# chao1224/pytorch_distributed_nn

Measured on AMD Instinct MI355X. Metric: samples/sec (whole node) ResNet-50 DDP, higher is better.
Workload: dtype bf16; 1 GPU; model=resnet50 (ImageNet layout, 224x224, 1000 classes), global_batch=256, per_gpu_batch=256, image_size=224, parallelism=dp1, optimizer=fused SGD momentum=0.9 wd=5e-5, hipgraph=False, opt_overlap=False

## Files before the change

csrc/kernels/conv1x1_wide.hip:

```cpp
#include "conv_direct.h"

namespace {
using namespace pg;

enum { PRE_NONE = 0, PRE_GM = 1 };
constexpr int W1_NB = 64;

template <int EPI, int PRE>
__global__ void __launch_bounds__(256, 2) conv1x1_wide_kernel(C3Args a) {
    constexpr int NB = W1_NB, FN = NB / 16;
    constexpr int BPT = NB * 8 / 256;
    extern __shared__ __attribute__((aligned(16))) char smem[];
    bf16_t* const bbuf = reinterpret_cast<bf16_t*>(smem);
    float* const coef = reinterpret_cast<float*>(bbuf + 2 * NB * 64);
    const int tid = threadIdx.x, lane = tid & 63, wave = tid >> 6;
    const int groups = a.ntiles;
    const int t = xcd_remap(blockIdx.x, a.tiles * groups);
    const int tile = t / groups, nt = t - tile * groups;
    const int p0 = tile * C3_BM, n0 = nt * NB;
    const int K = a.C, KC = K >> 6;

    u16x8_t rb[BPT];
    auto load_b = [&](int kc) {
#pragma unroll
// ... 105 lines not shown
}

template <int EPI, int PRE>
int wide_launch(const C3Args& a, hipStream_t st) {
    const int sm = 2 * W1_NB * 128 + (PRE != PRE_NONE ? 3 * a.C * 4 : 0);
    hipLaunchKernelGGL((conv1x1_wide_kernel<EPI, PRE>), dim3(a.tiles * a.ntiles), dim3(256), sm, st, a);
    PDNN_LAUNCH_RET;
}

template <int PRE>
int wide_dispatch(const C3Args& a, int epi, hipStream_t st) {
    switch (epi) {
        case C3_BNB: return wide_launch<C3_BNB, PRE>(a, st);
        case C3_STATS: return wide_launch<C3_STATS, PRE>(a, st);
        case C3_RES: return wide_launch<C3_RES, PRE>(a, st);
        default: return wide_launch<C3_PLAIN, PRE>(a, st);
    }
}

}

static FastDiv w1_fdiv(uint32_t d) {
    FastDiv f;
    f.d = d ? d : 1;
    uint32_t l = 0;
    while ((1ull << l) < f.d) ++l;
    f.s = l;
    f.m = (uint32_t)((((1ull << l) - f.d) << 32) / f.d + 1);
    return f;
}
// ... 14 lines not shown
    a.x = x; a.w = w; a.y = y; a.C = K; a.N = N; a.P = (int)P;
    a.dW = w1_fdiv(1); a.dH = w1_fdiv(1);
    a.stats = stats; a.res = res; a.rmask = res_mask;
    a.ep_x = bn_x; a.ep_mean = bn_mean; a.ep_invstd = bn_invstd; a.ep_mscale = bn_mscale; a.ep_mshift = bn_mshift;
    a.pre_t = pre_t; a.pre_mean = pre_mean; a.pre_invstd = pre_invstd; a.pre_gamma = pre_gamma;
    a.pre_dgamma = pre_dgamma; a.pre_dbeta = pre_dbeta; a.pre_out = pre_out;
    if (pre_t && !(pre_mean && pre_invstd && pre_dgamma && pre_dbeta)) return (int)hipErrorInvalidValue;
    if (pre_out && !pre_t) return (int)hipErrorInvalidValue;
    if (bn_x && !(bn_mean && bn_invstd && bn_mscale && bn_mshift)) return (int)hipErrorInvalidValue;
    const int epi = bn_x ? C3_BNB : (stats ? C3_STATS : (res ? C3_RES : C3_PLAIN));
    a.tiles = (int)cdiv(P, C3_BM);
    a.ntiles = N / W1_NB;
    if (pre_t) return wide_dispatch<PRE_GM>(a, epi, st);
    return wide_dispatch<PRE_NONE>(a, epi, st);
}
```

csrc/kernels/conv3x3.hip:

```cpp
#include "conv_direct.h"

namespace {
using namespace pg;

typedef __attribute__((ext_vector_type(8))) int c3v8i;
typedef __attribute__((ext_vector_type(4))) int c3v4i;
constexpr int C3_AMAX_PARTS = 1024;
#ifndef C3_PRE_J
#define C3_PRE_J 3
#endif
#ifndef C3_F8_PRE_J
#define C3_F8_PRE_J 2
#endif

template <int FMT>
__device__ __forceinline__ uint4 c3_to_fp8(const float* v) {
    constexpr float MX = FMT ? 57344.f : 448.f;
    int w[4];
#pragma unroll
    for (int d = 0; d < 4; ++d) {
        const float c0 = fminf(fmaxf(v[4 * d], -MX), MX), c1 = fminf(fmaxf(v[4 * d + 1], -MX), MX);
        const float c2 = fminf(fmaxf(v[4 * d + 2], -MX), MX), c3 = fminf(fmaxf(v[4 * d + 3], -MX), MX);
        int x = 0;
        if constexpr (FMT) {
// ... 616 lines not shown
}

template <int KC, int NB, bool PRE>
int areg_dispatch(const C3Args& a, int epi, hipStream_t st) {
    if constexpr (!PRE) {
        if (a.pro_sc) {
            if (epi == C3_STATS) return areg_launch<KC, NB, C3_STATS, false, true>(a, st);
            if (epi == C3_PLAIN) return areg_launch<KC, NB, C3_PLAIN, false, true>(a, st);
            return (int)hipErrorInvalidValue;
        }
    }
    switch (epi) {
        case C3_BNB: return areg_launch<KC, NB, C3_BNB, PRE>(a, st);
        case C3_STATS: return areg_launch<KC, NB, C3_STATS, PRE>(a, st);
        case C3_RES: return areg_launch<KC, NB, C3_RES, PRE>(a, st);
        default: return areg_launch<KC, NB, C3_PLAIN, PRE>(a, st);
    }
}

template <bool PRE>
int areg_run(C3Args& a, int K, int epi, hipStream_t st) {
    const int nb = K == 256 ? 32 : 64;
    const int chunks = a.N / nb;
    int g = 1;
    while (g < chunks && (long)a.tiles * g < 512 && chunks % (2 * g) == 0) g *= 2;
    a.ntiles = g;
    if (K == 64) return areg_dispatch<1, 64, PRE>(a, epi, st);
    if (K == 128) return areg_dispatch<2, 64, PRE>(a, epi, st);
    return areg_dispatch<4, 32, PRE>(a, epi, st);
}

static bool set_pre(C3Args& a, const bf16_t* t, const float* mean, const float* invstd, const float* gamma,
             const float* dgamma, const float* dbeta, bf16_t* out) {
    a.pre_t = t; a.pre_mean = mean; a.pre_invstd = invstd; a.pre_gamma = gamma;
    a.pre_dgamma = dgamma; a.pre_dbeta = dbeta; a.pre_out = out;
    if (!t) return !out;
    return mean && invstd && dgamma && dbeta;
}
static int c3_force() { return pg::tune().conv3x3_force; }

static FastDiv make_fdiv_c3(uint32_t d) {
    FastDiv f;
// ... 143 lines not shown
    if (!pdnn_conv1x1_panel_supported(P, K, N) || (bn_x && !stats) || (res_mask && !res) || (!pro_sc != !pro_sh) ||
        (pro_sc && (pre_t || bn_x || res)))
        return (int)hipErrorInvalidValue;
    C3Args a{};
    a.x = x; a.w = w; a.y = y; a.C = K; a.N = N; a.P = (int)P;
    a.tiles = (int)cdiv(P, C3_BM);
    a.stats = stats; a.res = res; a.rmask = res_mask;
    a.ep_x = bn_x; a.ep_mean = bn_mean; a.ep_invstd = bn_invstd; a.ep_mscale = bn_mscale; a.ep_mshift = bn_mshift;
    if (!set_pre(a, pre_t, pre_mean, pre_invstd, pre_gamma, pre_dgamma, pre_dbeta, pre_out))
        return (int)hipErrorInvalidValue;
    a.pro_sc = pro_sc; a.pro_sh = pro_sh;
    const int epi = bn_x ? C3_BNB : (stats ? C3_STATS : (res ? C3_RES : C3_PLAIN));
    return pre_t ? areg_run<true>(a, K, epi, st) : areg_run<false>(a, K, epi, st);
}

PDNN_API int pdnn_conv1x1_panel_stats_rows(long P) { return (int)cdiv(P, C3_BM) * 4; }
```

csrc/kernels/conv_direct.h:

```cpp
#pragma once
#include "gemm_common.h"
#include "tuning.h"

namespace {
using namespace pg;

constexpr int C3_BM = 256;
enum { C3_PLAIN = 0, C3_STATS = 1, C3_BNB = 2, C3_RES = 3 };

struct C3Args {
    const bf16_t* x;
    const bf16_t* w;
    bf16_t* y;
    int Nimg, H, W, C, N, P;
    FastDiv dW, dH;
    int tiles, ntiles;
    int halo_max;
    float* stats;
    const bf16_t* res;
    const uint8_t* rmask;
    const bf16_t* ep_x;
    const float *ep_mean, *ep_invstd, *ep_mscale, *ep_mshift;
    const bf16_t* pre_t;
    const float *pre_mean, *pre_invstd, *pre_gamma, *pre_dgamma, *pre_dbeta;
    bf16_t* pre_out;
    const float *f8_scale, *f8_inv, *f8_winv;
    float* f8_amax;
    const float *pro_sc, *pro_sh;
};

struct PreCoef {
    float k[8], A[8], B[8];
};
__device__ __forceinline__ void pre_coef(const C3Args& a, int c, PreCoef& pc) {
    const float invL = (float)(1.0 / (double)a.P);
// ... 68 lines not shown
    u.x &= m; u.y &= m; u.z &= m; u.w &= m;
    return __builtin_bit_cast(u16x8_t, u);
}

__device__ __forceinline__ u16x8_t c3_zero8() {
    u16x8_t z = {0, 0, 0, 0, 0, 0, 0, 0};
    return z;
}

__device__ __forceinline__ int halo_off(int hp, int q) {
    return hp * 64 + ((q ^ ((hp >> 1) & 7)) << 3);
}

template <int NB, int EPI>
struct C3PairOps {
    static constexpr bool RES = EPI == C3_RES, BNB = EPI == C3_BNB;
    u16x4_t tv[(RES || BNB) ? 2 : 1][4];
    uint32_t mw[RES ? 4 : 1];
};

template <int NB, int EPI>
__device__ __forceinline__ void c3_load_pair(const C3Args& a, const long (&lrow)[4], int n0, int lg, int fp,
                                             C3PairOps<NB, EPI>& o) {
    constexpr bool RES = EPI == C3_RES, BNB = EPI == C3_BNB;
    if constexpr (RES) {
#pragma unroll
        for (int fm = 0; fm < 4; ++fm)
            o.mw[fm] = a.rmask ? *reinterpret_cast<const uint32_t*>(a.rmask + ((lrow[fm] + n0 + 32 * fp) >> 3))
                               : 0xFFFFFFFFu;
    }
    if constexpr (RES || BNB) {
        const bf16_t* src = BNB ? a.ep_x : a.res;
#pragma unroll
        for (int h = 0; h < 2; ++h) {
            const int n = n0 + (2 * fp + h) * 16 + 4 * lg;
#pragma unroll
            for (int fm = 0; fm < 4; ++fm) o.tv[h][fm] = *reinterpret_cast<const u16x4_t*>(src + lrow[fm] + n);
        }
    }
}

template <int NB, int EPI>
__device__ __forceinline__ void c3_epilogue_rows(const C3Args& a, f32x4_t (&acc)[4][NB / 16], int tile,
                                                 const long (&orow)[4], int n0, int wave, int lane,
                                                 const bool (&pv)[4]) {
    constexpr int FN = NB / 16, NP = FN / 2;
    constexpr bool RES = EPI == C3_RES;
    const int lg = lane >> 4;
    long lrow[4];
#pragma unroll
    for (int fm = 0; fm < 4; ++fm) lrow[fm] = pv[fm] ? orow[fm] : 0;
    C3PairOps<NB, EPI> cur, nxt;
    if constexpr (NP > 1) c3_load_pair<NB, EPI>(a, lrow, n0, lg, 0, cur);
    else if constexpr (RES) {
#pragma unroll
        for (int fm = 0; fm < 4; ++fm)
            cur.mw[fm] = a.rmask ? *reinterpret_cast<const uint32_t*>(a.rmask + ((lrow[fm] + n0) >> 3)) : 0xFFFFFFFFu;
    }
#pragma unroll
    for (int fp = 0; fp < NP; ++fp) {
        if (fp + 1 < NP) c3_load_pair<NB, EPI>(a, lrow, n0, lg, fp + 1, nxt);
        uint32_t pk[4][2][2];
#pragma unroll
        for (int h = 0; h < 2; ++h) {
            const int fn = 2 * fp + h;
            const int n = n0 + fn * 16 + 4 * lg;
            float s[4] = {0, 0, 0, 0}, q[4] = {0, 0, 0, 0};
            float bms[4], bmh[4];
            if constexpr (NP == 1 && (RES || EPI == C3_BNB)) {
                const bf16_t* src = EPI == C3_BNB ? a.ep_x : a.res;
#pragma unroll
                for (int fm = 0; fm < 4; ++fm)
                    cur.tv[h][fm] = pv[fm] ? *reinterpret_cast<const u16x4_t*>(src + orow[fm] + n) : u16x4_t{0, 0, 0, 0};
            }
            if constexpr (EPI == C3_BNB) {
                const float4 m4 = *reinterpret_cast<const float4*>(a.ep_mscale + n);
                const float4 h4 = *reinterpret_cast<const float4*>(a.ep_mshift + n);
                bms[0] = m4.x; bms[1] = m4.y; bms[2] = m4.z; bms[3] = m4.w;
                bmh[0] = h4.x; bmh[1] = h4.y; bmh[2] = h4.z; bmh[3] = h4.w;
            }
#pragma unroll
            for (int fm = 0; fm < 4; ++fm) {
                const bool ok = pv[fm];
                float v[4];
#pragma unroll
                for (int j = 0; j < 4; ++j) v[j] = acc[fm][fn][j];
                if constexpr (RES) {
                    const uint32_t mb = cur.mw[fm] >> (16 * h + 4 * lg);
#pragma unroll
                    for (int j = 0; j < 4; ++j) v[j] += ((mb >> j) & 1) ? bf2f(cur.tv[h][fm][j]) : 0.f;
                }
                if constexpr (EPI == C3_BNB) {
#pragma unroll
                    for (int j = 0; j < 4; ++j) {
                        const float tt = bf2f(cur.tv[h][fm][j]);
                        const float gm = (ok && fmaf(tt, bms[j], bmh[j]) > 0.f) ? bf2f(f2bf(v[j])) : 0.f;
                        v[j] = gm;
                        s[j] += gm;
                        q[j] += gm * tt;
                    }
                } else if constexpr (EPI == C3_STATS) {
                    if (ok) {
#pragma unroll
                        for (int j = 0; j < 4; ++j) {
                            const float r = bf2f(f2bf(v[j]));
                            s[j] += r;
                            q[j] += r * r;
                        }
                    }
                }
                pk[fm][h][0] = pk2bf(v[0], v[1]);
                pk[fm][h][1] = pk2bf(v[2], v[3]);
            }
            if constexpr (EPI == C3_STATS || EPI == C3_BNB) {
#pragma unroll
                for (int j = 0; j < 4; ++j) {
                    s[j] = row16_sum(s[j]);
                    q[j] = row16_sum(q[j]);
                }
                {
                    float* ps = stat_row(a.stats, (long)tile * 4 + wave, a.N) + n;
                    if constexpr (EPI == C3_BNB) {
                        const int j = lane & 3;
                        if ((lane & 12) == 4) {
                            const float qj = (sel4(q, j) - a.ep_mean[n + j] * sel4(s, j)) * a.ep_invstd[n + j];
                            q[0] = q[1] = q[2] = q[3] = qj;
                        }
                    }
                    stat_add_frag(ps, ps + a.N, lane, s, q, true);
                }
            }
        }
#pragma unroll
        for (int fm = 0; fm < 4; ++fm) {
            const auto s0 = __builtin_amdgcn_permlane16_swap(pk[fm][0][0], pk[fm][1][0], false, false);
            const auto s1 = __builtin_amdgcn_permlane16_swap(pk[fm][0][1], pk[fm][1][1], false, false);
            const int n = n0 + (2 * fp + (lg & 1)) * 16 + 8 * (lg >> 1);
            if (pv[fm]) *reinterpret_cast<uint4*>(a.y + orow[fm] + n) = make_uint4(s0[0], s1[0], s0[1], s1[1]);
        }
        if (fp + 1 < NP) cur = nxt;
// ... 14 lines not shown
```

pytorch_distributed_nn_amd/ops/_backend.py:

```python
from __future__ import annotations

import ctypes
import functools
import os
from pathlib import Path

import torch

_LIBDIR = Path(__file__).resolve().parent.parent / "_lib"
_LIB = None
_ERR = None

P = ctypes.c_void_p
I = ctypes.c_int
L = ctypes.c_long
F = ctypes.c_float
D = ctypes.c_double

_SIGS = {
    "pdnn_gemm_nt": [P, L, P, L, P, L, I, I, I, F, P, I, I, P],
    "pdnn_gemm_nn": [P, L, P, L, P, L, I, I, I, F, I, P],
    "pdnn_gemm_tn_acc": [P, L, P, L, P, L, I, I, I, F, P],
    "pdnn_conv_fwd": [P, P, P, I, I, I, I, I, I, I, I, I, I, I, P, P, P, P],
    "pdnn_conv_dgrad": [P, P, P, I, I, I, I, I, I, I, I, I, I, I, P, P, P, P, P, P, P, P, P],
# ... 17 lines not shown
    "pdnn_conv3x3_wgrad_supported": [I, I, I, I, I],
    "pdnn_conv3x3_wgrad_ws": [I, I, I, I, I],
    "pdnn_conv3x3_force": [I],
    "pdnn_tune_set": [ctypes.c_char_p, I],
    "pdnn_tune_get": [ctypes.c_char_p],
    "pdnn_tune_list": [ctypes.c_char_p, I],
    "pdnn_tune_error": [],
    "pdnn_tune_unknown": [],
    "pdnn_set_comm_world": [I],
    "pdnn_grid_cus": [],
    "pdnn_conv1x1_panel": [P, P, P, L, I, I, P, P, P, P, P, P, P, P, P, P, P, P, P, P, P, P, P, P],
    "pdnn_conv1x1_panel_supported": [L, I, I],
    "pdnn_conv1x1_panel_stats_rows": [L],
    "pdnn_conv1x1_wide": [P, P, P, L, I, I] + [P] * 16,
    "pdnn_conv1x1_wide_supported": [L, I, I],
    "pdnn_stem_conv": [P, P, P, I, I, I, I, I, P, P],
    "pdnn_stem_stats_rows": [L],
    "pdnn_stem_conv_nchw": [P, P, P, I, I, I, I, I, P, P],
    "pdnn_stem_wgrad_nchw": [P, P, P, I, I, I, I, I, P, P, P, P, P, P, P, P, P, P, P],
    "pdnn_stem_wgrad_ws": [I, I, I],
    "pdnn_bn_relu_maxpool": [P, P, P, P, P, I, I, I, I, I, I, P],
    "pdnn_set_glds_mode": [I],
    "pdnn_set_pp_mode": [I],
    "pdnn_set_pp_bn": [I],
    "pdnn_set_pp_trace": [P],
    "pdnn_pp_wgrad": [P, L, P, L, P, L, I, I, I, F, P, I, P, I, P],
    "pdnn_pp_wgrad_plan": [I, I, I, I],
    "pdnn_pp_wgrad_splits": [I, I, I],
    "pdnn_pp_wgrad_ws": [I, I, I],
    "pdnn_pp_wgrad_splits_long": [I, I, I],
# ... 188 lines not shown
```

pytorch_distributed_nn_amd/ops/fused_resnet.py:

```python
from __future__ import annotations

import contextlib
import os

import torch

from .. import tuning
from ..optim.flat import SHADOW_EPOCH, direct_grad, grad_ready
from . import kernels as K
from .functional import weight_bf16

F32 = torch.float32


def _bn_train(slab, M, bn_params, bufs, mom, eps):
    gamma, beta = bn_params
    rm, rv = bufs
    rows = slab.shape[0] // 2
    return K.bn_finalize(slab, rows, M, eps, mom, gamma, beta, rm, rv)


def _bn_eval(bn_params, bufs, eps):
    gamma, beta = bn_params
    rm, rv = bufs
# ... 140 lines not shown


def _bn_back(g2d, t2d, mean, inv, gamma, mode, msrc=None, msc=None, msh=None, sink=None, bn_params=None):
    slab, _, rows = K.bn_bwd_reduce(g2d, t2d, mean, inv, mode=mode, msrc=msrc, mscale=msc, mshift=msh)
    if sink is not None:
        (dgamma, dbeta), (rg, rb) = sink.bn(slab, rows, *bn_params)
        dt, _, _ = K.bn_bwd_apply(g2d, t2d, mean, inv, gamma, dgamma, dbeta, mode=mode, msrc=msrc, mscale=msc,
                                  mshift=msh)
        return dt, rg, rb
    dgamma, dbeta = K.bn_bwd_finalize(slab, rows)
    dt, _, _ = K.bn_bwd_apply(g2d, t2d, mean, inv, gamma, dgamma, dbeta, mode=mode, msrc=msrc, mscale=msc,
                              mshift=msh)
    return dt, dgamma, dbeta


def _dgrad_bn_gm(dy, wk, t, st, pad, mean, inv, sc, sh, sink, gamma_p, beta_p, wprep=None):
    gm, slab = K.conv_dgrad(dy, wk, t.shape, st, pad, bn=(t, mean, inv, sc, sh), wprep=wprep)
    (dgamma, dbeta), ret = sink.bn(slab, slab.shape[0] // 2, gamma_p, beta_p)
    return gm, dgamma, dbeta, ret


_FWD_FORKED = {}
_WPREP_SEQ = [0]
_WPREP_WAITED = {}


@contextlib.contextmanager
def side_forward(dev):
    side = _side_stream(dev) if dev.type == "cuda" else None
    if side is None:
        yield
        return
    K.stream_wait(side, torch.cuda.current_stream(dev))
    _FWD_FORKED[dev.index] = SHADOW_EPOCH[0]
    try:
        yield
    finally:
        _FWD_FORKED.pop(dev.index, None)


def _wait_wprep(dev, ev, seq):
    if _WPREP_WAITED.get(dev.index, -1) >= seq:
        return
# ... 17 lines not shown
        ev.record(side)
    for sp, w in zip(specs, ws):
        if sp is None:
            continue
        sp[1].record_stream(side)
        if w is not None:
            w.record_stream(main)
    _WPREP_SEQ[0] += 1
    return ws, (ev, _WPREP_SEQ[0])


def _pre_ok(t, wk, st, pad):
    return K.dgrad_pre_ok(tuple(t.shape), tuple(wk.shape), st, pad)


def _fused_dgrad_bn(dy, wk, t, st, pad, mean, inv, sc, sh, gamma, sink, gamma_p, beta_p, wprep=None):
    gm, slab = K.conv_dgrad(dy, wk, t.shape, st, pad, bn=(t, mean, inv, sc, sh), wprep=wprep)
    (dgamma, dbeta), ret = sink.bn(slab, slab.shape[0] // 2, gamma_p, beta_p)
    C = t.shape[-1]
    dt, _, _ = K.bn_bwd_apply(gm.view(-1, C), t.view(-1, C), mean, inv, gamma, dgamma, dbeta, mode=0)
    return dt.view(t.shape), ret[0], ret[1]


def _krsc_grad(dw):
    return dw.permute(0, 3, 1, 2)


class BottleneckFn(torch.autograd.Function):

    @staticmethod
    def forward(ctx, x, conf, bufs, shadows, *params):
        stride, training, mom, eps = conf[:4]
        fp8_meta = conf[4] if len(conf) > 4 else None
        down = len(params) == 12
        w1, g1, b1, w2, g2, b2, w3, g3, b3 = params[:9]
        k1, k2, k3 = shadows[:3]
        side_down = None
        xd = x
        side = _side_stream(x.device) if down else None
        if side is not None:
            main = torch.cuda.current_stream(x.device)
            K.stream_wait(side, main)
            with torch.cuda.stream(side):
                side_down, xd = _shortcut_fwd(x, shadows[3], stride, training, (params[10], params[11]), bufs[6:8],
                                              mom, eps)
            x.record_stream(side)
            for t in side_down + (xd,):
                t.record_stream(main)
        t1, m1, i1, s1, h1 = _conv_bn(x, k1, 1, 0, None, training, (g1, b1), bufs[0:2], mom, eps)
        C1 = t1.shape[-1]
        if stride == 1 and K.conv3x3_pro_ok(tuple(t1.shape), w2.shape[0]):
# ... 29 lines not shown
        t3, m3, i3, s3, h3 = _conv_bn(src2, k3, 1, 0, pro2, training, (g3, b3), bufs[4:6], mom, eps)
        C3 = t3.shape[-1]
        if down:
            if side_down is not None:
                K.stream_wait(main, side)
                td, md, idd, sd, hd = side_down
            else:
                (td, md, idd, sd, hd), xd = _shortcut_fwd(x, shadows[3], stride, training, (params[10], params[11]),
                                                          bufs[6:8], mom, eps)
            out, mb = K.bn_apply(t3.view(-1, C3), s3, h3, res=td.view(-1, C3), rscale=sd, rshift=hd, relu=True,
                                 want_mask=training)
        else:
            td = md = idd = None
            out, mb = K.bn_apply(t3.view(-1, C3), s3, h3, res=x.view(-1, C3), relu=True, want_mask=training)
        out = out.view(t3.shape)
        ctx.wprep = None
        if training:
            ctx.wprep = _prep_dgrad_weights(x, [(tuple(t3.shape), k3, tuple(t2.shape), 1, 0),
                                                (tuple(t2.shape), k2, tuple(t1.shape), stride, 1) if fp8 is None
                                                else None,
                                                (tuple(t1.shape), k1, tuple(x.shape), 1, 0)])
        ctx.save_for_backward(x, t1, a1, t2, t3, td, mb, m1, i1, s1, h1, m2, i2, s2, h2, m3, i3, md, idd,
                              g1, g2, g3, params[10] if down else None, k1, k2, k3, shadows[3] if down else None, a2,
                              xd if (down and xd is not x) else None)
        ctx.conf = (stride, training, down)
        ctx.params = params
        ctx.fp8 = fp8
        return out

    @staticmethod
    def backward(ctx, gout):
        (x, t1, a1, t2, t3, td, mb, m1, i1, s1, h1, m2, i2, s2, h2, m3, i3, md, idd,
         g1, g2, g3, gd, k1, k2, k3, kd, a2, xs) = ctx.saved_tensors
        stride, training, down = ctx.conf
        if not training:
            raise RuntimeError("fused Bottleneck backward requires training-mode BatchNorm")
        gout = gout.contiguous()
        C3 = t3.shape[-1]
        g2d, t3_2d = gout.view(-1, C3), t3.view(-1, C3)
        P = ctx.params
        ctx.params = None
        sink = _Sink(gout.device)
        w3p = w2p = w1p = None
        if ctx.wprep is not None:
            (w3p, w2p, w1p), (ev, seq) = ctx.wprep
            _wait_wprep(gout.device, ev, seq)
            ctx.wprep = None
        gres_mask = mb if MASKED_RES else None
        slab3, slabd, rows = K.bn_bwd_reduce(g2d, t3_2d, m3, i3, mode=3, msrc=mb,
                                             x2=td.view(-1, C3) if down else None, mean2=md, invstd2=idd)
        (dg3, db3), (rg3, rb3) = sink.bn(slab3, rows, P[7], P[8])
        if down:
            (dgd, dbd), (rgd, rbd) = sink.bn(slabd, rows, P[10], P[11])
            dt3, dtd, _ = K.bn_bwd_apply(g2d, t3_2d, m3, i3, g3, dg3, db3, mode=3, msrc=mb,
                                         x2=td.view(-1, C3), mean2=md, invstd2=idd, gamma2=gd, dgamma2=dgd,
                                         dbeta2=dbd)
            gres = None
        elif MASKED_RES:
            dt3, _, _ = K.bn_bwd_apply(g2d, t3_2d, m3, i3, g3, dg3, db3, mode=3, msrc=mb)
            gres = gout
        else:
            dt3, _, gres = K.bn_bwd_apply(g2d, t3_2d, m3, i3, g3, dg3, db3, mode=3, msrc=mb, want_gm=True)
        dt3 = dt3.view(t3.shape)
        dw3 = sink.wgrad(P[6], a2 if a2 is not None else t2, dt3, 1, 1, 1, 0, pro=None if a2 is not None else (s2, h2))
        bn1 = (t1, m1, i1, s1, h1)
        if _pre_ok(t2, k2, stride, 1):
            gm2, dg2, db2, (rg2, rb2) = _dgrad_bn_gm(dt3, k3, t2, 1, 0, m2, i2, s2, h2, sink, P[4], P[5], wprep=w3p)
            dt2 = torch.empty_like(t2)
            pre2 = (t2, m2, i2, g2, dg2, db2, dt2)
            if ctx.fp8 is not None:
                from .fp8 import weight_fp8_flip
                wt8, winv = weight_fp8_flip(P[3])
                gm1, slab1 = K.conv3x3_fp8(gm2, wt8, winv, ctx.fp8.bwd, bn=bn1, pre=pre2)
            else:
                gm1, slab1 = K.conv_dgrad(gm2, k2, t1.shape, stride, 1, bn=bn1, pre=pre2, wprep=w2p)
            del gm2
            dw2 = sink.wgrad(P[3], a1 if a1 is not None else t1, dt2, 3, 3, stride, 1,
                             pro=None if a1 is not None else (s1, h1), fp8=ctx.fp8)
        else:
            dt2, rg2, rb2 = _fused_dgrad_bn(dt3, k3, t2, 1, 0, m2, i2, s2, h2, g2, sink, P[4], P[5], wprep=w3p)
            dw2 = sink.wgrad(P[3], a1 if a1 is not None else t1, dt2, 3, 3, stride, 1,
                             pro=None if a1 is not None else (s1, h1))
            gm1, slab1 = K.conv_dgrad(dt2, k2, t1.shape, stride, 1, bn=bn1, wprep=w2p)
        (dg1, db1), (rg1, rb1) = sink.bn(slab1, slab1.shape[0] // 2, P[1], P[2])
        pre1 = None
        if _pre_ok(t1, k1, 1, 0):
            dt1 = torch.empty_like(t1)
            pre1 = (t1, m1, i1, g1, dg1, db1, dt1)
            dy1 = gm1
        else:
            C1 = t1.shape[-1]
            dt1 = K.bn_bwd_apply(gm1.view(-1, C1), t1.view(-1, C1), m1, i1, g1, dg1, db1, mode=0)[0].view(t1.shape)
            dw1 = sink.wgrad(P[0], x, dt1, 1, 1, 1, 0)
            dy1 = dt1
        if down:
            dtd = dtd.view(td.shape)
            dwd = sink.wgrad(P[9], xs, dtd, 1, 1, 1, 0) if xs is not None else sink.wgrad(P[9], x, dtd, 1, 1, stride, 0)
            dx = K.conv_dgrad(dy1, k1, x.shape, 1, 0, pre=pre1, wprep=w1p)
            dx = K.conv_dgrad(dtd, kd, x.shape, stride, 0, res=dx, out=dx)
        else:
            dx = K.conv_dgrad(dy1, k1, x.shape, 1, 0, res=gres.view(x.shape), res_mask=gres_mask, pre=pre1,
                              wprep=w1p)
        if pre1 is not None:
            dw1 = sink.wgrad(P[0], x, dt1, 1, 1, 1, 0)
        grads = (dw1, rg1, rb1, dw2, rg2, rb2, dw3, rg3, rb3) + ((dwd, rgd, rbd) if down else ())
        sink.done()
        return (dx, None, None, None) + grads


class BasicBlockFn(torch.autograd.Function):

    @staticmethod
    def forward(ctx, x, conf, bufs, shadows, *params):
        stride, training, mom, eps = conf
# ... 162 lines not shown
```

pytorch_distributed_nn_amd/ops/kernels.py:

```python
from __future__ import annotations

import ctypes

import torch

from ._backend import _CUR_DEV, call, lib, ptr, stream

BF16 = torch.bfloat16
F32 = torch.float32


def _chk(cond, msg):
    if not cond:
        raise ValueError(msg)


def _is_krsc(w):
    K, C, R, S = w.shape
    return w.stride() == (R * S * C, 1, S * C, C)


def _bf16_c(t, name):
    _chk(t.dtype == BF16 and t.is_cuda, f"{name}: expected CUDA bf16, got {t.dtype} {t.device}")
    _chk(t.is_contiguous(), f"{name}: expected contiguous tensor")
# ... 238 lines not shown
    return (_P1["mode"] and R == 1 and S == 1 and st == 1 and pad == 0
            and (lib().pdnn_conv1x1_panel_supported(P, K, N) == 1 or _wide_ok(P, K, N, fwd)))


def _pre_args(pre, x):
    if pre is None:
        return (None,) * 7
    t, mean, inv, gamma, dg, db, dt_out = pre
    _bf16_c(t, "pre.t")
    _chk(t.numel() == x.numel(), "pre: t must have the operand's shape")
    if dt_out is not None:
        _chk(dt_out.numel() == x.numel() and dt_out.dtype == BF16 and dt_out.is_contiguous(), "pre: dt_out")
    return tuple(ptr(v) for v in (t, mean, inv, gamma, dg, db, dt_out))


def conv1x1_panel(x2d, w2d, want_stats=False, res=None, bn=None, res_mask=None, out=None, pre=None, pro=None):
    P, Kc = x2d.shape
    N = w2d.shape[0]
    y = out if out is not None else torch.empty(P, N, device=x2d.device, dtype=BF16)
    slab = None
    t = mean = inv = msc = msh = None
    if want_stats or bn is not None:
        slab = stat_bins(N, x2d.device)
    if bn is not None:
        t, mean, inv, msc, msh = bn
    if Kc >= 512:
        _chk(pro is None, "conv1x1_panel: the forward prologue needs K <= 256")
        call("pdnn_conv1x1_wide", ptr(x2d), ptr(w2d), ptr(y), P, Kc, N, ptr(slab), ptr(res), ptr(res_mask), ptr(t),
             ptr(mean), ptr(inv), ptr(msc), ptr(msh), *_pre_args(pre, x2d), stream())
        return y, slab
    psc, psh = pro if pro is not None else (None, None)
    call("pdnn_conv1x1_panel", ptr(x2d), ptr(w2d), ptr(y), P, Kc, N, ptr(slab), ptr(res), ptr(res_mask), ptr(t),
         ptr(mean), ptr(inv), ptr(msc), ptr(msh), *_pre_args(pre, x2d), ptr(psc), ptr(psh), stream())
    return y, slab
# ... 57 lines not shown


def conv3x3_pro_ok(x_shape, Ko):
    N, H, W, C = x_shape
    return _conv3x3_ok(N, H, W, C, Ko, 3, 3, 1, 1) and lib().pdnn_conv3x3_wgrad_supported(N, H, W, C, Ko) == 1


def dgrad_pre_ok(dy_shape, w_shape, st, pad):
    N, Ho, Wo, K = dy_shape
    Kw, R, S, C = w_shape
    return (_conv3x3_ok(N, Ho, Wo, K, C, R, S, st, pad)
            or (_s2_ok(N, 2 * Ho, 2 * Wo, C, K, R, S, st, pad, 1) and (_tuning.get("s2_halo") & 16) != 0)
            or (_panel_dgrad_k(K) and _panel_ok(N * Ho * Wo, K, C, R, S, st, pad)))


def dgrad_weight(dy_shape, w, x_shape, st, pad):
    N, Ho, Wo, K = dy_shape
    _, H, W, C = x_shape
    Kw, R, S, C2 = w.shape
    if _conv3x3_ok(N, Ho, Wo, K, C, R, S, st, pad) or _s2_ok(N, H, W, C, K, R, S, st, pad, 1):
        return conv3x3_flip(w)
    if _panel_dgrad_k(K) and _panel_ok(N * H * W, K, C, R, S, st, pad):
        return transpose_bf16(w.view(K, C))
    return None


def conv_dgrad(dy, w, x_shape, st, pad, res=None, bn=None, out=None, res_mask=None, pre=None, wprep=None):
    _bf16_c(dy, "conv_dgrad.dy")
    N, H, W, C = x_shape
    _bf16_c(w, "conv_dgrad.w")
    K, R, S, C2 = w.shape
    _chk(C2 == C, "conv_dgrad: weight [K][R][S][C]")
    _, Ho, Wo, K2 = dy.shape
    _chk(K2 == K and C % 8 == 0 and K % 8 == 0, "conv_dgrad: channel mismatch")
    if out is not None:
        _chk(tuple(out.shape) == (N, H, W, C) and out.dtype == BF16 and out.is_contiguous(), "conv_dgrad: out")
        _chk(bn is None, "conv_dgrad: out with a fused BN backward")
    if bn is not None:
        _bf16_c(bn[0], "conv_dgrad.bn_x")
        _chk(tuple(bn[0].shape) == (N, H, W, C), "conv_dgrad: bn_x shape")
    if res is not None:
        _bf16_c(res, "conv_dgrad.res")
        _chk(tuple(res.shape) == (N, H, W, C), "conv_dgrad: res shape")
    if res_mask is not None:
        _chk(res is not None and st == 1 and res_mask.dtype == torch.uint8 and res_mask.is_contiguous()
             and res_mask.numel() * 8 == N * H * W * C and (out is None or out.data_ptr() != res.data_ptr()),
             "conv_dgrad: res_mask needs res, stride 1, uint8 [N*H*W][C/8], out not aliasing res")
    if _conv3x3_ok(N, Ho, Wo, K, C, R, S, st, pad):
        y, slab = conv3x3(dy, wprep if wprep is not None else conv3x3_flip(w), res=res, bn=bn, out=out,
                          res_mask=res_mask, pre=pre)
        return (y, slab) if bn is not None else y
    if _s2_ok(N, H, W, C, K, R, S, st, pad, 1) and res is None and out is None and (H, W) == (2 * Ho, 2 * Wo):
        y, slab = conv3x3s2(dy, wprep if wprep is not None else conv3x3_flip(w), dgrad=True, bn=bn, pre=pre)
        return (y, slab) if bn is not None else y
    if _panel_dgrad_k(K) and _panel_ok(N * H * W, K, C, R, S, st, pad) and (out is None or res is not None):
        y, slab = conv1x1_panel(dy.view(-1, K), wprep if wprep is not None else transpose_bf16(w.view(K, C)),
                                res=None if res is None else res.view(-1, C), res_mask=res_mask,
                                bn=None if bn is None else (bn[0].view(-1, C),) + tuple(bn[1:]),
                                out=None if out is None else out.view(-1, C), pre=pre)
        y = y.view(N, H, W, C)
        return (y, slab) if bn is not None else y
    _chk(pre is None, "conv_dgrad: pre= needs the halo 3x3 or K = 64 panel kernel (dgrad_pre_ok)")
# ... 768 lines not shown
```

pytorch_distributed_nn_amd/tuning.py:

```python
from __future__ import annotations

import os

DEFAULTS = {"side_wgrad": 1, "wide1x1_dgrad": 1, "a2_fold": 1, "wt_prefetch": 0, "wt_layer_batch": 1, "colsum_atomic": 1, "bias_in_wgrad": 1, "s2_halo": 3, "ds_sub": 1, "wgrad1x1_pp_pix": 200704, "gpt2_side_wgrad": 1, "xent_fused": 1, "wgrad_plan_cus": 128}

_VALUES = dict(DEFAULTS)


def _parse(s: str) -> dict:
    out = {}
    for item in filter(None, (p.strip() for p in s.split(","))):
        if "=" not in item:
            raise ValueError(f"PDNN_TUNE: {item!r} is not key=value")
        k, v = item.split("=", 1)
        out[k.strip()] = int(v)
    return out


for _k, _v in _parse(os.environ.get("PDNN_TUNE", "")).items():
    if _k in _VALUES:
        _VALUES[_k] = _v


def get(key: str) -> int:
# ... 10 lines not shown
```

Before: 12240 samples/s.

## Fuse next block's BN3 backward reduction into previous block's conv1 dgrad epilogue

Adds a RES_BNB epilogue to the 1x1 panel and wide dgrad kernels. It applies the following block's ReLU sign bits, adds the residual gradient and accumulates that block's BN3 dgamma/dbeta partial sums while writing dx. The forward pass records (t3, mean, invstd, mask) keyed by the block output, and the backward pass reuses the fused stats slab in the next bottleneck, skipping a separate bn_bwd_reduce pass over gout. It also lets conv3's dgrad apply the BN3 backward as a prologue ('pre'). The cost is extra mask and t loads in the epilogue plus id/weakref bookkeeping, enabled per stage width by the bn3_fuse bitmask.

```diff
diff --git a/csrc/kernels/conv1x1_wide.hip b/csrc/kernels/conv1x1_wide.hip
--- a/csrc/kernels/conv1x1_wide.hip
+++ b/csrc/kernels/conv1x1_wide.hip
@@ -143,6 +143,7 @@
         case C3_BNB: return wide_launch<C3_BNB, PRE>(a, st);
         case C3_STATS: return wide_launch<C3_STATS, PRE>(a, st);
         case C3_RES: return wide_launch<C3_RES, PRE>(a, st);
+        case C3_RES_BNB: return wide_launch<C3_RES_BNB, PRE>(a, st);
         default: return wide_launch<C3_PLAIN, PRE>(a, st);
     }
 }
@@ -187,3 +188,26 @@
     if (pre_t) return wide_dispatch<PRE_GM>(a, epi, st);
     return wide_dispatch<PRE_NONE>(a, epi, st);
 }
+
+PDNN_API int pdnn_conv1x1_wide_bnbits(const bf16_t* x, const bf16_t* w, bf16_t* y, long P, int K, int N, float* stats,
+                                      const bf16_t* res, const uint8_t* res_mask, const bf16_t* bn_t,
+                                      const float* bn_mean, const float* bn_invstd, const uint8_t* bn_bits,
+                                      const bf16_t* pre_t, const float* pre_mean, const float* pre_invstd,
+                                      const float* pre_gamma, const float* pre_dgamma, const float* pre_dbeta,
+                                      bf16_t* pre_out, hipStream_t st) {
+    if (!pdnn_conv1x1_wide_supported(P, K == 256 ? 512 : K, N) || !stats || !res || !bn_t || !bn_mean || !bn_invstd ||
+        !bn_bits)
+        return (int)hipErrorInvalidValue;
+    if (pre_t && !(pre_mean && pre_invstd && pre_dgamma && pre_dbeta)) return (int)hipErrorInvalidValue;
+    if (pre_out && !pre_t) return (int)hipErrorInvalidValue;
+    C3Args a{};
+    a.x = x; a.w = w; a.y = y; a.C = K; a.N = N; a.P = (int)P;
+    a.dW = w1_fdiv(1); a.dH = w1_fdiv(1);
+    a.stats = stats; a.res = res; a.rmask = res_mask; a.bmask = bn_bits;
+    a.ep_x = bn_t; a.ep_mean = bn_mean; a.ep_invstd = bn_invstd;
+    a.pre_t = pre_t; a.pre_mean = pre_mean; a.pre_invstd = pre_invstd; a.pre_gamma = pre_gamma;
+    a.pre_dgamma = pre_dgamma; a.pre_dbeta = pre_dbeta; a.pre_out = pre_out;
+    a.tiles = (int)cdiv(P, C3_BM);
+    a.ntiles = N / W1_NB;
+    return pre_t ? wide_dispatch<PRE_GM>(a, C3_RES_BNB, st) : wide_dispatch<PRE_NONE>(a, C3_RES_BNB, st);
+}
diff --git a/csrc/kernels/conv3x3.hip b/csrc/kernels/conv3x3.hip
--- a/csrc/kernels/conv3x3.hip
+++ b/csrc/kernels/conv3x3.hip
@@ -654,18 +654,24 @@
         case C3_BNB: return areg_launch<KC, NB, C3_BNB, PRE>(a, st);
         case C3_STATS: return areg_launch<KC, NB, C3_STATS, PRE>(a, st);
         case C3_RES: return areg_launch<KC, NB, C3_RES, PRE>(a, st);
+        case C3_RES_BNB:
+            if constexpr ((KC == 1 && NB == 64) || (KC == 2 && NB == 32))
+                return areg_launch<KC, NB, C3_RES_BNB, PRE>(a, st);
+            else
+                return (int)hipErrorInvalidValue;
         default: return areg_launch<KC, NB, C3_PLAIN, PRE>(a, st);
     }
 }
 
 template <bool PRE>
 int areg_run(C3Args& a, int K, int epi, hipStream_t st) {
-    const int nb = K == 256 ? 32 : 64;
+    const int nb = (K == 256 || (K == 128 && epi == C3_RES_BNB)) ? 32 : 64;
     const int chunks = a.N / nb;
     int g = 1;
     while (g < chunks && (long)a.tiles * g < 512 && chunks % (2 * g) == 0) g *= 2;
     a.ntiles = g;
     if (K == 64) return areg_dispatch<1, 64, PRE>(a, epi, st);
+    if (K == 128 && epi == C3_RES_BNB) return areg_launch<2, 32, C3_RES_BNB, PRE>(a, st);
     if (K == 128) return areg_dispatch<2, 64, PRE>(a, epi, st);
     return areg_dispatch<4, 32, PRE>(a, epi, st);
 }
@@ -839,4 +845,30 @@
     return pre_t ? areg_run<true>(a, K, epi, st) : areg_run<false>(a, K, epi, st);
 }
 
+PDNN_API int pdnn_conv1x1_wide_supported(long P, int K, int N);
+
+PDNN_API int pdnn_conv1x1_bnbits_supported(long P, int K, int N) {
+    if (K == 64 || K == 128) return pdnn_conv1x1_panel_supported(P, K, N);
+    return K == 256 ? pdnn_conv1x1_wide_supported(P, 512, N) : pdnn_conv1x1_wide_supported(P, K, N);
+}
+
+PDNN_API int pdnn_conv1x1_panel_bnbits(const bf16_t* x, const bf16_t* w, bf16_t* y, long P, int K, int N,
+                                       float* stats, const bf16_t* res, const uint8_t* res_mask, const bf16_t* bn_t,
+                                       const float* bn_mean, const float* bn_invstd, const uint8_t* bn_bits,
+                                       const bf16_t* pre_t, const float* pre_mean, const float* pre_invstd,
+                                       const float* pre_gamma, const float* pre_dgamma, const float* pre_dbeta,
+                                       bf16_t* pre_out, hipStream_t st) {
+    if (!pdnn_conv1x1_panel_supported(P, K, N) || K == 256 || !stats || !res || !bn_t || !bn_mean || !bn_invstd ||
+        !bn_bits)
+        return (int)hipErrorInvalidValue;
+    C3Args a{};
+    a.x = x; a.w = w; a.y = y; a.C = K; a.N = N; a.P = (int)P;
+    a.tiles = (int)cdiv(P, C3_BM);
+    a.stats = stats; a.res = res; a.rmask = res_mask; a.bmask = bn_bits;
+    a.ep_x = bn_t; a.ep_mean = bn_mean; a.ep_invstd = bn_invstd;
+    if (!set_pre(a, pre_t, pre_mean, pre_invstd, pre_gamma, pre_dgamma, pre_dbeta, pre_out))
+        return (int)hipErrorInvalidValue;
+    return pre_t ? areg_run<true>(a, K, C3_RES_BNB, st) : areg_run<false>(a, K, C3_RES_BNB, st);
+}
+
 PDNN_API int pdnn_conv1x1_panel_stats_rows(long P) { return (int)cdiv(P, C3_BM) * 4; }
diff --git a/csrc/kernels/conv_direct.h b/csrc/kernels/conv_direct.h
--- a/csrc/kernels/conv_direct.h
+++ b/csrc/kernels/conv_direct.h
@@ -6,7 +6,7 @@
 using namespace pg;
 
 constexpr int C3_BM = 256;
-enum { C3_PLAIN = 0, C3_STATS = 1, C3_BNB = 2, C3_RES = 3 };
+enum { C3_PLAIN = 0, C3_STATS = 1, C3_BNB = 2, C3_RES = 3, C3_RES_BNB = 4 };
 
 struct C3Args {
     const bf16_t* x;
@@ -19,6 +19,7 @@
     float* stats;
     const bf16_t* res;
     const uint8_t* rmask;
+    const uint8_t* bmask;
     const bf16_t* ep_x;
     const float *ep_mean, *ep_invstd, *ep_mscale, *ep_mshift;
     const bf16_t* pre_t;
@@ -117,21 +118,28 @@
 
 template <int NB, int EPI>
 struct C3PairOps {
-    static constexpr bool RES = EPI == C3_RES, BNB = EPI == C3_BNB;
+    static constexpr bool RB = EPI == C3_RES_BNB, RES = EPI == C3_RES || RB, BNB = EPI == C3_BNB;
     u16x4_t tv[(RES || BNB) ? 2 : 1][4];
     uint32_t mw[RES ? 4 : 1];
+    u16x4_t tt[RB ? 2 : 1][4];
+    uint32_t bw[RB ? 4 : 1];
 };
 
 template <int NB, int EPI>
 __device__ __forceinline__ void c3_load_pair(const C3Args& a, const long (&lrow)[4], int n0, int lg, int fp,
                                              C3PairOps<NB, EPI>& o) {
-    constexpr bool RES = EPI == C3_RES, BNB = EPI == C3_BNB;
+    constexpr bool RB = EPI == C3_RES_BNB, RES = EPI == C3_RES || RB, BNB = EPI == C3_BNB;
     if constexpr (RES) {
 #pragma unroll
         for (int fm = 0; fm < 4; ++fm)
             o.mw[fm] = a.rmask ? *reinterpret_cast<const uint32_t*>(a.rmask + ((lrow[fm] + n0 + 32 * fp) >> 3))
                                : 0xFFFFFFFFu;
     }
+    if constexpr (RB) {
+#pragma unroll
+        for (int fm = 0; fm < 4; ++fm)
+            o.bw[fm] = *reinterpret_cast<const uint32_t*>(a.bmask + ((lrow[fm] + n0 + 32 * fp) >> 3));
+    }
     if constexpr (RES || BNB) {
         const bf16_t* src = BNB ? a.ep_x : a.res;
 #pragma unroll
@@ -139,6 +147,11 @@
             const int n = n0 + (2 * fp + h) * 16 + 4 * lg;
 #pragma unroll
             for (int fm = 0; fm < 4; ++fm) o.tv[h][fm] = *reinterpret_cast<const u16x4_t*>(src + lrow[fm] + n);
+            if constexpr (RB) {
+#pragma unroll
+                for (int fm = 0; fm < 4; ++fm)
+                    o.tt[h][fm] = *reinterpret_cast<const u16x4_t*>(a.ep_x + lrow[fm] + n);
+            }
         }
     }
 }
@@ -148,7 +161,7 @@
                                                  const long (&orow)[4], int n0, int wave, int lane,
                                                  const bool (&pv)[4]) {
     constexpr int FN = NB / 16, NP = FN / 2;
-    constexpr bool RES = EPI == C3_RES;
+    constexpr bool RB = EPI == C3_RES_BNB, RES = EPI == C3_RES || RB;
     const int lg = lane >> 4;
     long lrow[4];
 #pragma unroll
@@ -159,6 +172,11 @@
 #pragma unroll
         for (int fm = 0; fm < 4; ++fm)
             cur.mw[fm] = a.rmask ? *reinterpret_cast<const uint32_t*>(a.rmask + ((lrow[fm] + n0) >> 3)) : 0xFFFFFFFFu;
+        if constexpr (RB) {
+#pragma unroll
+            for (int fm = 0; fm < 4; ++fm)
+                cur.bw[fm] = *reinterpret_cast<const uint32_t*>(a.bmask + ((lrow[fm] + n0) >> 3));
+        }
     }
 #pragma unroll
     for (int fp = 0; fp < NP; ++fp) {
@@ -170,11 +188,22 @@
             const int n = n0 + fn * 16 + 4 * lg;
             float s[4] = {0, 0, 0, 0}, q[4] = {0, 0, 0, 0};
             float bms[4], bmh[4];
+            [[maybe_unused]] float bmu[4];
+            if constexpr (RB) {
+                const float4 u4 = *reinterpret_cast<const float4*>(a.ep_mean + n);
+                bmu[0] = u4.x; bmu[1] = u4.y; bmu[2] = u4.z; bmu[3] = u4.w;
+            }
             if constexpr (NP == 1 && (RES || EPI == C3_BNB)) {
                 const bf16_t* src = EPI == C3_BNB ? a.ep_x : a.res;
 #pragma unroll
                 for (int fm = 0; fm < 4; ++fm)
                     cur.tv[h][fm] = pv[fm] ? *reinterpret_cast<const u16x4_t*>(src + orow[fm] + n) : u16x4_t{0, 0, 0, 0};
+                if constexpr (RB) {
+#pragma unroll
+                    for (int fm = 0; fm < 4; ++fm)
+                        cur.tt[h][fm] = pv[fm] ? *reinterpret_cast<const u16x4_t*>(a.ep_x + orow[fm] + n)
+                                               : u16x4_t{0, 0, 0, 0};
+                }
             }
             if constexpr (EPI == C3_BNB) {
                 const float4 m4 = *reinterpret_cast<const float4*>(a.ep_mscale + n);
@@ -193,7 +222,17 @@
 #pragma unroll
                     for (int j = 0; j < 4; ++j) v[j] += ((mb >> j) & 1) ? bf2f(cur.tv[h][fm][j]) : 0.f;
                 }
-                if constexpr (EPI == C3_BNB) {
+                if constexpr (RB) {
+                    const uint32_t bb = cur.bw[fm] >> (16 * h + 4 * lg);
+#pragma unroll
+                    for (int j = 0; j < 4; ++j) {
+                        const float tt = bf2f(cur.tt[h][fm][j]);
+                        const float gm = (ok && ((bb >> j) & 1)) ? bf2f(f2bf(v[j])) : 0.f;
+                        v[j] = gm;
+                        s[j] += gm;
+                        q[j] += gm * (tt - bmu[j]);
+                    }
+                } else if constexpr (EPI == C3_BNB) {
 #pragma unroll
                     for (int j = 0; j < 4; ++j) {
                         const float tt = bf2f(cur.tv[h][fm][j]);
@@ -215,7 +254,7 @@
                 pk[fm][h][0] = pk2bf(v[0], v[1]);
                 pk[fm][h][1] = pk2bf(v[2], v[3]);
             }
-            if constexpr (EPI == C3_STATS || EPI == C3_BNB) {
+            if constexpr (EPI == C3_STATS || EPI == C3_BNB || RB) {
 #pragma unroll
                 for (int j = 0; j < 4; ++j) {
                     s[j] = row16_sum(s[j]);
@@ -223,10 +262,11 @@
                 }
                 {
                     float* ps = stat_row(a.stats, (long)tile * 4 + wave, a.N) + n;
-                    if constexpr (EPI == C3_BNB) {
+                    if constexpr (EPI == C3_BNB || RB) {
                         const int j = lane & 3;
                         if ((lane & 12) == 4) {
-                            const float qj = (sel4(q, j) - a.ep_mean[n + j] * sel4(s, j)) * a.ep_invstd[n + j];
+                            const float qj = RB ? sel4(q, j) * a.ep_invstd[n + j]
+                                                : (sel4(q, j) - a.ep_mean[n + j] * sel4(s, j)) * a.ep_invstd[n + j];
                             q[0] = q[1] = q[2] = q[3] = qj;
                         }
                     }
diff --git a/pytorch_distributed_nn_amd/ops/_backend.py b/pytorch_distributed_nn_amd/ops/_backend.py
--- a/pytorch_distributed_nn_amd/ops/_backend.py
+++ b/pytorch_distributed_nn_amd/ops/_backend.py
@@ -55,6 +55,9 @@
     "pdnn_conv1x1_panel_stats_rows": [L],
     "pdnn_conv1x1_wide": [P, P, P, L, I, I] + [P] * 16,
     "pdnn_conv1x1_wide_supported": [L, I, I],
+    "pdnn_conv1x1_bnbits_supported": [L, I, I],
+    "pdnn_conv1x1_panel_bnbits": [P, P, P, L, I, I] + [P] * 15,
+    "pdnn_conv1x1_wide_bnbits": [P, P, P, L, I, I] + [P] * 15,
     "pdnn_stem_conv": [P, P, P, I, I, I, I, I, P, P],
     "pdnn_stem_stats_rows": [L],
     "pdnn_stem_conv_nchw": [P, P, P, I, I, I, I, I, P, P],
diff --git a/pytorch_distributed_nn_amd/ops/fused_resnet.py b/pytorch_distributed_nn_amd/ops/fused_resnet.py
--- a/pytorch_distributed_nn_amd/ops/fused_resnet.py
+++ b/pytorch_distributed_nn_amd/ops/fused_resnet.py
@@ -2,6 +2,8 @@
 
 import contextlib
 import os
+import sys
+import weakref
 
 import torch
 
@@ -178,8 +180,8 @@
     return dt, dgamma, dbeta
 
 
-def _dgrad_bn_gm(dy, wk, t, st, pad, mean, inv, sc, sh, sink, gamma_p, beta_p, wprep=None):
-    gm, slab = K.conv_dgrad(dy, wk, t.shape, st, pad, bn=(t, mean, inv, sc, sh), wprep=wprep)
+def _dgrad_bn_gm(dy, wk, t, st, pad, mean, inv, sc, sh, sink, gamma_p, beta_p, wprep=None, pre=None):
+    gm, slab = K.conv_dgrad(dy, wk, t.shape, st, pad, bn=(t, mean, inv, sc, sh), wprep=wprep, pre=pre)
     (dgamma, dbeta), ret = sink.bn(slab, slab.shape[0] // 2, gamma_p, beta_p)
     return gm, dgamma, dbeta, ret
 
@@ -191,6 +193,7 @@
 
 @contextlib.contextmanager
 def side_forward(dev):
+    _bn3_clear()
     side = _side_stream(dev) if dev.type == "cuda" else None
     if side is None:
         yield
@@ -238,12 +241,46 @@
     return K.dgrad_pre_ok(tuple(t.shape), tuple(wk.shape), st, pad)
 
 
-def _fused_dgrad_bn(dy, wk, t, st, pad, mean, inv, sc, sh, gamma, sink, gamma_p, beta_p, wprep=None):
-    gm, slab = K.conv_dgrad(dy, wk, t.shape, st, pad, bn=(t, mean, inv, sc, sh), wprep=wprep)
+def _fused_dgrad_bn(dy, wk, t, st, pad, mean, inv, sc, sh, gamma, sink, gamma_p, beta_p, wprep=None, pre=None):
+    gm, slab = K.conv_dgrad(dy, wk, t.shape, st, pad, bn=(t, mean, inv, sc, sh), wprep=wprep, pre=pre)
     (dgamma, dbeta), ret = sink.bn(slab, slab.shape[0] // 2, gamma_p, beta_p)
     C = t.shape[-1]
     dt, _, _ = K.bn_bwd_apply(gm.view(-1, C), t.view(-1, C), mean, inv, gamma, dgamma, dbeta, mode=0)
     return dt.view(t.shape), ret[0], ret[1]
+
+
+_BN3_FWD = {}
+_BN3_BWD = {}
+
+
+def bn3_records():
+    return len(_BN3_FWD), len(_BN3_BWD)
+
+
+def _bn3_clear():
+    _BN3_FWD.clear()
+    _BN3_BWD.clear()
+
+
+def _bn3_put(table, tensor, payload):
+    key = id(tensor)
+    table[key] = (weakref.ref(tensor, lambda _r, k=key, t=table: t.pop(k, None)),) + payload
+
+
+def _bn3_take(table, tensor):
+    rec = table.get(id(tensor))
+    if rec is None:
+        return None
+    del table[id(tensor)]
+    return rec[1:] if rec[0]() is tensor else None
+
+
+def _bn3_observed(t):
+    return bool(getattr(t, "_backward_hooks", None)) or bool(getattr(t, "retains_grad", False))
+
+
+def _bn3_stage_on(width):
+    return (tuning.get("bn3_fuse") >> (max(width // 64, 1).bit_length() - 1)) & 1 == 1
 
 
 def _krsc_grad(dw):
@@ -259,6 +296,12 @@
         down = len(params) == 12
         w1, g1, b1, w2, g2, b2, w3, g3, b3 = params[:9]
         k1, k2, k3 = shadows[:3]
+        bn3_src = _bn3_take(_BN3_FWD, x)
+        fuse3 = training and not down and stride == 1 and _bn3_stage_on(w1.shape[0])
+        if not (fuse3 and bn3_src is not None and not _bn3_observed(x) and K.dgrad_bn_bits_ok(
+                tuple(x.shape[:3]) + (k1.shape[0],), tuple(k1.shape), 1, 0)):
+            bn3_src = None
+        ctx.bn3_src = bn3_src
         side_down = None
         xd = x
         side = _side_stream(x.device) if down else None
@@ -318,6 +361,8 @@
             td = md = idd = None
             out, mb = K.bn_apply(t3.view(-1, C3), s3, h3, res=x.view(-1, C3), relu=True, want_mask=training)
         out = out.view(t3.shape)
+        if fuse3 and mb is not None:
+            _bn3_put(_BN3_FWD, out, (t3, m3, i3, mb))
         ctx.wprep = None
         if training:
             ctx.wprep = _prep_dgrad_weights(x, [(tuple(t3.shape), k3, tuple(t2.shape), 1, 0),
@@ -334,11 +379,22 @@
 
     @staticmethod
     def backward(ctx, gout):
+        if not ctx.conf[1]:
+            raise RuntimeError("fused Bottleneck backward requires training-mode BatchNorm")
+        bn3_src, ctx.bn3_src = ctx.bn3_src, None
+        bn3_done = _bn3_take(_BN3_BWD, gout)
+        try:
+            return BottleneckFn._backward(ctx, gout, bn3_src, bn3_done)
+        finally:
+            _BN3_FWD.clear()
+            if sys.exc_info()[0] is not None:
+                _BN3_BWD.clear()
+
+    @staticmethod
+    def _backward(ctx, gout, bn3_src, bn3_done):
         (x, t1, a1, t2, t3, td, mb, m1, i1, s1, h1, m2, i2, s2, h2, m3, i3, md, idd,
          g1, g2, g3, gd, k1, k2, k3, kd, a2, xs) = ctx.saved_tensors
         stride, training, down = ctx.conf
-        if not training:
-            raise RuntimeError("fused Bottleneck backward requires training-mode BatchNorm")
         gout = gout.contiguous()
         C3 = t3.shape[-1]
         g2d, t3_2d = gout.view(-1, C3), t3.view(-1, C3)
@@ -351,25 +407,45 @@
             _wait_wprep(gout.device, ev, seq)
             ctx.wprep = None
         gres_mask = mb if MASKED_RES else None
-        slab3, slabd, rows = K.bn_bwd_reduce(g2d, t3_2d, m3, i3, mode=3, msrc=mb,
-                                             x2=td.view(-1, C3) if down else None, mean2=md, invstd2=idd)
-        (dg3, db3), (rg3, rb3) = sink.bn(slab3, rows, P[7], P[8])
-        if down:
-            (dgd, dbd), (rgd, rbd) = sink.bn(slabd, rows, P[10], P[11])
-            dt3, dtd, _ = K.bn_bwd_apply(g2d, t3_2d, m3, i3, g3, dg3, db3, mode=3, msrc=mb,
-                                         x2=td.view(-1, C3), mean2=md, invstd2=idd, gamma2=gd, dgamma2=dgd,
-                                         dbeta2=dbd)
-            gres = None
-        elif MASKED_RES:
-            dt3, _, _ = K.bn_bwd_apply(g2d, t3_2d, m3, i3, g3, dg3, db3, mode=3, msrc=mb)
-            gres = gout
-        else:
-            dt3, _, gres = K.bn_bwd_apply(g2d, t3_2d, m3, i3, g3, dg3, db3, mode=3, msrc=mb, want_gm=True)
+        pre3 = None
+        if bn3_done is not None:
+            (slab3,) = bn3_done
+            (dg3, db3), (rg3, rb3) = sink.bn(slab3, slab3.shape[0] // 2, P[7], P[8])
+            if (tuning.get("bn3_fuse") & 16) and _pre_ok(t3, k3, 1, 0):
+                dt3 = torch.empty_like(t3)
+                pre3 = (t3, m3, i3, g3, dg3, db3, dt3)
+            else:
+                dt3, _, _ = K.bn_bwd_apply(g2d, t3_2d, m3, i3, g3, dg3, db3, mode=0)
+            gres, gres_mask = gout, None
+        else:
+            slab3, slabd, rows = K.bn_bwd_reduce(g2d, t3_2d, m3, i3, mode=3, msrc=mb,
+                                                 x2=td.view(-1, C3) if down else None, mean2=md, invstd2=idd)
+            (dg3, db3), (rg3, rb3) = sink.bn(slab3, rows, P[7], P[8])
+            if down:
+                (dgd, dbd), (rgd, rbd) = sink.bn(slabd, rows, P[10], P[11])
+                dt3, dtd, _ = K.bn_bwd_apply(g2d, t3_2d, m3, i3, g3, dg3, db3, mode=3, msrc=mb,
+                                             x2=td.view(-1, C3), mean2=md, invstd2=idd, gamma2=gd, dgamma2=dgd,
+                                             dbeta2=dbd)
+                gres = None
+            elif MASKED_RES:
+                dt3, _, _ = K.bn_bwd_apply(g2d, t3_2d, m3, i3, g3, dg3, db3, mode=3, msrc=mb)
+                gres = gout
+            else:
+                dt3, _, gres = K.bn_bwd_apply(g2d, t3_2d, m3, i3, g3, dg3, db3, mode=3, msrc=mb, want_gm=True)
         dt3 = dt3.view(t3.shape)
-        dw3 = sink.wgrad(P[6], a2 if a2 is not None else t2, dt3, 1, 1, 1, 0, pro=None if a2 is not None else (s2, h2))
+
+        def wgrad3():
+            return sink.wgrad(P[6], a2 if a2 is not None else t2, dt3, 1, 1, 1, 0,
+                              pro=None if a2 is not None else (s2, h2))
+        dy3 = dt3 if pre3 is None else gout
+        if pre3 is None:
+            dw3 = wgrad3()
         bn1 = (t1, m1, i1, s1, h1)
         if _pre_ok(t2, k2, stride, 1):
-            gm2, dg2, db2, (rg2, rb2) = _dgrad_bn_gm(dt3, k3, t2, 1, 0, m2, i2, s2, h2, sink, P[4], P[5], wprep=w3p)
+            gm2, dg2, db2, (rg2, rb2) = _dgrad_bn_gm(dy3, k3, t2, 1, 0, m2, i2, s2, h2, sink, P[4], P[5], wprep=w3p,
+                                                     pre=pre3)
+            if pre3 is not None:
+                dw3 = wgrad3()
             dt2 = torch.empty_like(t2)
             pre2 = (t2, m2, i2, g2, dg2, db2, dt2)
             if ctx.fp8 is not None:
@@ -382,7 +458,10 @@
             dw2 = sink.wgrad(P[3], a1 if a1 is not None else t1, dt2, 3, 3, stride, 1,
                              pro=None if a1 is not None else (s1, h1), fp8=ctx.fp8)
         else:
-            dt2, rg2, rb2 = _fused_dgrad_bn(dt3, k3, t2, 1, 0, m2, i2, s2, h2, g2, sink, P[4], P[5], wprep=w3p)
+            dt2, rg2, rb2 = _fused_dgrad_bn(dy3, k3, t2, 1, 0, m2, i2, s2, h2, g2, sink, P[4], P[5], wprep=w3p,
+                                            pre=pre3)
+            if pre3 is not None:
+                dw3 = wgrad3()
             dw2 = sink.wgrad(P[3], a1 if a1 is not None else t1, dt2, 3, 3, stride, 1,
                              pro=None if a1 is not None else (s1, h1))
             gm1, slab1 = K.conv_dgrad(dt2, k2, t1.shape, stride, 1, bn=bn1, wprep=w2p)
@@ -402,6 +481,10 @@
             dwd = sink.wgrad(P[9], xs, dtd, 1, 1, 1, 0) if xs is not None else sink.wgrad(P[9], x, dtd, 1, 1, stride, 0)
             dx = K.conv_dgrad(dy1, k1, x.shape, 1, 0, pre=pre1, wprep=w1p)
             dx = K.conv_dgrad(dtd, kd, x.shape, stride, 0, res=dx, out=dx)
+        elif bn3_src is not None and not _bn3_observed(x):
+            dx, slab_up = K.conv_dgrad(dy1, k1, x.shape, 1, 0, res=gres.view(x.shape), res_mask=gres_mask, pre=pre1,
+                                       wprep=w1p, bn_bits=bn3_src)
+            _bn3_put(_BN3_BWD, dx, (slab_up,))
         else:
             dx = K.conv_dgrad(dy1, k1, x.shape, 1, 0, res=gres.view(x.shape), res_mask=gres_mask, pre=pre1,
                               wprep=w1p)
diff --git a/pytorch_distributed_nn_amd/ops/kernels.py b/pytorch_distributed_nn_amd/ops/kernels.py
--- a/pytorch_distributed_nn_amd/ops/kernels.py
+++ b/pytorch_distributed_nn_amd/ops/kernels.py
@@ -276,10 +276,19 @@
     return tuple(ptr(v) for v in (t, mean, inv, gamma, dg, db, dt_out))
 
 
-def conv1x1_panel(x2d, w2d, want_stats=False, res=None, bn=None, res_mask=None, out=None, pre=None, pro=None):
+def conv1x1_panel(x2d, w2d, want_stats=False, res=None, bn=None, res_mask=None, out=None, pre=None, pro=None,
+                  bn_bits=None):
     P, Kc = x2d.shape
     N = w2d.shape[0]
     y = out if out is not None else torch.empty(P, N, device=x2d.device, dtype=BF16)
+    if bn_bits is not None:
+        _chk(bn is None and pro is None and not want_stats, "conv1x1_panel: bn_bits excludes bn / pro / want_stats")
+        t, mean, inv, bits = bn_bits
+        slab = stat_bins(N, x2d.device)
+        call("pdnn_conv1x1_wide_bnbits" if Kc >= 256 else "pdnn_conv1x1_panel_bnbits", ptr(x2d), ptr(w2d), ptr(y), P,
+             Kc, N, ptr(slab), ptr(res), ptr(res_mask), ptr(t), ptr(mean), ptr(inv), ptr(bits), *_pre_args(pre, x2d),
+             stream())
+        return y, slab
     slab = None
     t = mean = inv = msc = msh = None
     if want_stats or bn is not None:
@@ -367,6 +376,27 @@
             or (_panel_dgrad_k(K) and _panel_ok(N * Ho * Wo, K, C, R, S, st, pad)))
 
 
+def dgrad_bn_bits_ok(dy_shape, w_shape, st, pad):
+    N, Ho, Wo, K = dy_shape
+    Kw, R, S, C = w_shape
+    P = N * Ho * Wo
+    return bool(_panel_dgrad_k(K) and _panel_ok(P, K, C, R, S, st, pad)
+                and lib().pdnn_conv1x1_bnbits_supported(P, K, C) == 1)
+
+
+def _bn_bits_args(bn_bits, L, C, name):
+    _chk(len(bn_bits) == 4, f"{name}: bn_bits = (t, mean, invstd, bits)")
+    t, mean, inv, bits = bn_bits
+    _bn_c(C, name)
+    _bf16_c(t, f"{name}: bn_bits t")
+    _chk(t.numel() == L * C and t.shape[-1] == C, f"{name}: bn_bits t must be [{L}][{C}]")
+    _bn_vec(mean, C, f"{name}: bn_bits mean")
+    _bn_vec(inv, C, f"{name}: bn_bits invstd")
+    _chk(bits is not None and bits.dtype == torch.uint8 and bits.is_cuda and bits.is_contiguous()
+         and bits.numel() * 8 == L * C, f"{name}: bn_bits bits must be bn_apply's uint8 [{L}][{C // 8}] sign bits")
+    return t.view(-1, C), mean, inv, bits
+
+
 def dgrad_weight(dy_shape, w, x_shape, st, pad):
     N, Ho, Wo, K = dy_shape
     _, H, W, C = x_shape
@@ -378,7 +408,8 @@
     return None
 
 
-def conv_dgrad(dy, w, x_shape, st, pad, res=None, bn=None, out=None, res_mask=None, pre=None, wprep=None):
+def conv_dgrad(dy, w, x_shape, st, pad, res=None, bn=None, out=None, res_mask=None, pre=None, wprep=None,
+               bn_bits=None):
     _bf16_c(dy, "conv_dgrad.dy")
     N, H, W, C = x_shape
     _bf16_c(w, "conv_dgrad.w")
@@ -399,6 +430,17 @@
         _chk(res is not None and st == 1 and res_mask.dtype == torch.uint8 and res_mask.is_contiguous()
              and res_mask.numel() * 8 == N * H * W * C and (out is None or out.data_ptr() != res.data_ptr()),
              "conv_dgrad: res_mask needs res, stride 1, uint8 [N*H*W][C/8], out not aliasing res")
+    if bn_bits is not None:
+        _chk(bn is None and res is not None and (out is None or out.data_ptr() != res.data_ptr()),
+             "conv_dgrad: bn_bits needs res, excludes bn and out aliasing res")
+        _chk(dgrad_bn_bits_ok(tuple(dy.shape), tuple(w.shape), st, pad),
+             "conv_dgrad: bn_bits= needs a 1x1 / stride-1 data gradient on the A-stationary or long-reduction kernel "
+             "(dgrad_bn_bits_ok)")
+        y, slab = conv1x1_panel(dy.view(-1, K), wprep if wprep is not None else transpose_bf16(w.view(K, C)),
+                                res=res.view(-1, C), res_mask=res_mask, pre=pre,
+                                out=None if out is None else out.view(-1, C),
+                                bn_bits=_bn_bits_args(bn_bits, N * H * W, C, "conv_dgrad"))
+        return y.view(N, H, W, C), slab
     if _conv3x3_ok(N, Ho, Wo, K, C, R, S, st, pad):
         y, slab = conv3x3(dy, wprep if wprep is not None else conv3x3_flip(w), res=res, bn=bn, out=out,
                           res_mask=res_mask, pre=pre)
diff --git a/pytorch_distributed_nn_amd/tuning.py b/pytorch_distributed_nn_amd/tuning.py
--- a/pytorch_distributed_nn_amd/tuning.py
+++ b/pytorch_distributed_nn_amd/tuning.py
@@ -2,7 +2,7 @@
 
 import os
 
-DEFAULTS = {"side_wgrad": 1, "wide1x1_dgrad": 1, "a2_fold": 1, "wt_prefetch": 0, "wt_layer_batch": 1, "colsum_atomic": 1, "bias_in_wgrad": 1, "s2_halo": 3, "ds_sub": 1, "wgrad1x1_pp_pix": 200704, "gpt2_side_wgrad": 1, "xent_fused": 1, "wgrad_plan_cus": 128}
+DEFAULTS = {"side_wgrad": 1, "wide1x1_dgrad": 1, "a2_fold": 1, "wt_prefetch": 0, "wt_layer_batch": 1, "colsum_atomic": 1, "bias_in_wgrad": 1, "s2_halo": 3, "ds_sub": 1, "wgrad1x1_pp_pix": 200704, "gpt2_side_wgrad": 1, "xent_fused": 1, "wgrad_plan_cus": 128, "bn3_fuse": 25}
 
 _VALUES = dict(DEFAULTS)
 
```

Measured after the change: 12230 samples/s. Within noise of the previous version (-0.1%).
